# vpc-ccg/tksm

Measured on AMD Instinct MI355X. Metric: sequenced reads/s, higher is better.
Workload: dtype u8; 1 GPU; Bulk molecules, Badread error+qual model (nanopore2020, identity 84,99,5.5), 24 x 128 Mb random genome, FASTQ; kind=bulk, mean_len=1000, length_distribution=normal(1000, 200), compute_qual=True, contexts_in_flight_per_gpu=3

## Files before the change

### tksm_amd/csrc/kernels.hip

```cpp
#include "kernels.h"
#include <type_traits>

namespace tk {

#define DEV __device__ __forceinline__

constexpr int BIG = 1 << 28;
DEV bool is_inf(int v) { return v >= (1 << 27); }

struct Ph4 { uint32_t x, y, z, w; };
enum { ST_ID = 0, ST_PAD = 1, ST_IDENT = 2, ST_DRAW = 3, ST_ALNPOS = 4, ST_QUAL = 5, ST_TAIL = 6 };

DEV Ph4 philox(uint64_t seed, uint64_t read, uint32_t stream, uint32_t n) {
    uint32_t c0 = (uint32_t)read, c1 = (uint32_t)(read >> 32), c2 = stream, c3 = n;
    uint32_t k0 = (uint32_t)seed, k1 = (uint32_t)(seed >> 32);
#pragma unroll
    for (int r = 0; r < 10; r++) {
        const unsigned long long p0 = (unsigned long long)0xD2511F53u * c0, p1 = (unsigned long long)0xCD9E8D57u * c2;
        const uint32_t h0 = (uint32_t)(p0 >> 32), l0 = (uint32_t)p0, h1 = (uint32_t)(p1 >> 32), l1 = (uint32_t)p1;
        uint32_t n0 = h1 ^ c1 ^ k0, n2 = h0 ^ c3 ^ k1;
        c0 = n0; c1 = l1; c2 = n2; c3 = l0;
        k0 += 0x9E3779B9u; k1 += 0xBB67AE85u;
    }
    return Ph4{c0, c1, c2, c3};
// ... 1542 lines not shown
            }
            wave_sync();
            const int m = join_window_planar(gnb, p0, nrows, Nw, ownw, wcap, lane);
            wave_sync();
            if (m > wcap) {
                if (early_mode) { to_exact_kernel(); return; }
                break;
            }
            const AlnOut a = band_align<0, false>(Fw, nrows, Nw, ownw, m, lane, nullptr);
            st_aligns++;
            if (is_inf(a.dist)) {
                to_exact_kernel();
                return;
            }
            const int cols = (int)(a.stat & 0xffffu), mt = (int)(a.stat >> 16);
            const double ident = cols ? (double)mt / (double)cols : 0.0;
            if (L <= 1000) errors = (1.0 - ident) * frag_len;
            else {
                const double estimated = (1.0 - ident) * frag_len;
                const double weight = 1000.0 / frag_len;
                errors = estimated * weight + errors * (1.0 - weight);
            }
            aln_no++;
            st = RUN;
        }
    }
    if (lane == 0) {
        uint32_t job = 0;
        if (st == NEED_ALN) {
            job = FB.base_cur[rc] + atomicAdd(&FB.job_cnt[rc * 32u], 1u);
            st_aligns++;
            uint32_t p0 = 0, nrows = (uint32_t)L;
            if (L > 1000) {
                p0 = __umulhi(philox(P.seed, g, ST_ALNPOS, aln_no).x, (uint32_t)(L - 1000 + 1));
                nrows = 1000u;
            }
            *reinterpret_cast<uint4*>(FB.job_meta + 4ull * job) = make_uint4(r, p0, nrows, 0u);
        }
        sp->errors = errors; sp->est = est_keep; sp->change_count = change_count; sp->n_base = n; sp->aln_no = aln_no;
        sp->resume_src = -1; sp->resume_j = (int16_t)resume_j; sp->st_draws = st_draws; sp->st_aligns = st_aligns;
        sp->pending = st == NEED_ALN ? 1 : 0;
        sp->job = job;
        sp->stage = st == NEED_ALN ? 0 : 3;
        if (st == DONE) {
            atomicAdd(&FB.defer_cnt[rc * 32u], 1u);
            FB.defer_list[atomicAdd(&FB.counters[1], 1u)] = make_uint2(r, rc);
        }
    }
}

template <bool STATE_IN_HBM>
__global__ __launch_bounds__(256, 8) void k_err(BatchView B, ErrModelView EM, QsModelView QM, SimParams P, SimBuffers O,
                                              FastBuffers FB, const uint32_t* __restrict__ order, uint32_t begin, uint32_t count,
                                              int lds_lcap, int lds_ncap, int from_jobs, uint32_t c0, uint32_t c1) {
#ifndef TKSM_ABLATE
    __builtin_amdgcn_s_setprio(2);
#endif
    const int lane = threadIdx.x & 63, wave = __builtin_amdgcn_readfirstlane(threadIdx.x >> 6), wpw = blockDim.x >> 6;
    const uint32_t widx = blockIdx.x * (uint32_t)wpw + (uint32_t)wave;
    if (widx >= count) return;
    uint64_t r; uint32_t pos;
    if (!from_jobs) { pos = begin + widx; r = (uint64_t)__builtin_amdgcn_readfirstlane((int)order[pos]) & 0xffffffffull; }
    else if (from_jobs == 2) {
        const uint2 e = FB.defer_list[widx];
        r = (uint64_t)__builtin_amdgcn_readfirstlane((int)e.x) & 0xffffffffull;
        pos = (uint32_t)__builtin_amdgcn_readfirstlane((int)e.y) * FB.rs;
    } else {
        const uint32_t target = FB.prefix[c0] + widx;
        uint32_t lo2 = c0, hi2 = c1 - 1;
        while (lo2 < hi2) { const uint32_t mid = (lo2 + hi2 + 1) >> 1; if (FB.prefix[mid] <= target) lo2 = mid; else hi2 = mid - 1; }
        const uint32_t pjob = FB.base_prev[lo2] + (target - FB.prefix[lo2]);
        r = (uint64_t)__builtin_amdgcn_readfirstlane((int)FB.prev_meta[4ull * pjob]) & 0xffffffffull;
        pos = lo2 * FB.rs;
    }
    ReadState S = FB.state[r];
    if (S.stage == 2 || S.slow) return;
    if (S.stage == 0) return;
    uint16_t* gnb = nb_row(FB, r);
    const int per_wave = STATE_IN_HBM ? lds_ncap + 128 : lds_lcap * 3 + lds_ncap + 128;
    uint8_t* lds_wave = lds_raw + (size_t)wave * per_wave;
    uint8_t* frag = STATE_IN_HBM ? frag_row(FB, r) : lds_wave;
    uint16_t* nb = STATE_IN_HBM ? gnb : reinterpret_cast<uint16_t*>(lds_wave + lds_lcap);
    uint8_t* aux = STATE_IN_HBM ? lds_wave : lds_wave + 3 * (size_t)lds_lcap;
    const int k = EM.k;
    const uint64_t g = P.first_read + r * P.stride;
    const int raw_len = __builtin_amdgcn_readfirstlane(S.raw_len);
    const int L = raw_len + 2 * k;
    const uint64_t slot = O.slot_off[r];
    const int cap = __builtin_amdgcn_readfirstlane((int)((O.slot_off[r + 1] - slot) >> 1));
    uint8_t* out_seq = O.scratch + slot;
    uint8_t* out_qual = out_seq + cap;
    if (!STATE_IN_HBM) {
        const uint8_t* gfrag0 = frag_row(FB, r);
        for (int t = lane * 4; t < L; t += 256) *reinterpret_cast<uint32_t*>(frag + t) = *reinterpret_cast<const uint32_t*>(gfrag0 + t);
        for (int t = lane * 2; t < L; t += 128) *reinterpret_cast<uint32_t*>(nb + t) = *reinterpret_cast<const uint32_t*>(gnb + t);
    }
    wave_sync();
    uint32_t status = 0;
    const double frag_len = (double)L;
    const double errors = S.errors;
    const double target = S.target;
    const int change_count = __builtin_amdgcn_readfirstlane(S.change_count), st_draws = __builtin_amdgcn_readfirstlane(S.st_draws);
    int st_aligns = __builtin_amdgcn_readfirstlane(S.st_aligns);
    double identity = 1.0;

    int start_trim, end_trim;
    {
        int v1 = lane < k ? slot_len(nb[lane]) : 0, v2 = lane < k ? slot_len(nb[L - k + lane]) : 0;
        (void)prefix_small(v1, start_trim);
        (void)prefix_small(v2, end_trim);
    }
    const int jcap = min(lds_ncap, cap);
    const int m = joined_len(nb, 0, L, lane);
    int lo = start_trim, hi = end_trim == 0 ? 0 : m - end_trim;
    lo = min(lo, m); hi = max(hi, lo);
    if (m > jcap) { status |= 1; lo = hi = 0; }
    const int out_len = hi - lo;
    const bool want_q = P.compute_q && m > 0 && !(status & 1);
    if (want_q) {
        const uint32_t mt = S.res_mt, cols = S.res_cols, fail = S.res_fail;
        if (fail) { go_slow(FB, r, lane, 3); return; }
        identity = cols ? (double)mt / (double)cols : 0.0;
        const uint32_t rc1 = pos / FB.rs;
        const uint8_t* gp = FB.prev_popd + FB.geo_prev[rc1].popd_off + (size_t)(S.job - FB.base_prev[rc1]) * FB.geo_prev[rc1].ncap;
        wave_sync();
        uint8_t* popd = aux + 16;
        for (int t = lane; t < m; t += 64) popd[t] = gp[t];
        wave_sync();
        const int margins = (QM.kmer_size - 1) / 2;
        const uint32_t hmask = (uint32_t)QM.n_slots - 1u;
        for (int i2 = lo + lane; i2 < hi; i2 += 64) {
#ifdef TKSM_ABLATE
            if (P.ablate == 40) { out_qual[i2 - lo] = 40; continue; }
#endif
            const int d = max(0, max(margins - i2, i2 + margins - (m - 1)));
            int row = -1; uint32_t roff = 0, rcnt = 0;
            auto probe = [&](uint64_t key) {
                uint32_t sl = (uint32_t)qs_hash(key) & hmask;
#ifdef TKSM_ABLATE
                if (P.ablate == 41) { row = (int)(sl & 1023u); roff = 0u; rcnt = 1u; return; }
#endif
                for (;;) {
                    const uint4 e = QM.ent[sl];
                    const uint64_t kk = ((uint64_t)e.y << 32) | e.x;
                    if (kk == key) { row = (int)sl; roff = e.z; rcnt = e.w; break; }
                    if (kk == 0) break;
                    sl = (sl + 1) & hmask;
                }
            };
            if (margins <= 4) {
                const int ob = 16 + i2 - 4, sh = ob & 3;
                const uint32_t* aw = reinterpret_cast<const uint32_t*>(aux) + (ob >> 2);
                const uint32_t w0 = aw[0], w1 = aw[1], w2 = aw[2];
                const uint32_t b0 = __builtin_amdgcn_alignbyte(w1, w0, sh), b1 = __builtin_amdgcn_alignbyte(w2, w1, sh), b2 = w2 >> (8 * sh);
                auto byte_at = [&](int j) -> uint32_t { return j < 4 ? (b0 >> (8 * j)) & 255u : j < 8 ? (b1 >> (8 * (j - 4))) & 255u : b2 & 255u; };
                uint64_t K[5]; int ln[5];
                K[0] = byte_at(4) & 3u; ln[0] = 1;
#pragma unroll
                for (int h = 1; h <= 4; h++) {
                    const uint32_t bl = byte_at(4 - h);
                    const int ddl = (int)(bl >> 2), ddr = (int)(byte_at(3 + h) >> 2);
                    ln[h] = ln[h - 1] + 2 + ddl + ddr;
                    const bool fits = ln[h] <= 29;
                    const int sl_ = fits ? 2 * (1 + ddl) : 0, sr_ = fits ? 2 * (1 + ddl + ln[h - 1]) : 0, so_ = fits ? 2 * (ln[h] - 1) : 0;
                    const int dl2 = fits ? 2 * ddl : 0, dr2 = fits ? 2 * ddr : 0;
                    K[h] = (uint64_t)(bl & 3u) | (((1ull << dl2) - 1ull) << 2) | (K[h - 1] << sl_) | (((1ull << dr2) - 1ull) << sr_) |
                           ((uint64_t)(byte_at(4 + h) & 3u) << so_);
                }
                const int hmax = margins - d;
                bool pend = true;
#pragma unroll
                for (int h = 4; h >= 0; h--) {
                    const bool tryit = pend && h <= hmax;
                    if (__ballot(tryit) == 0ull) continue;
                    if (tryit && ln[h] <= 29) { probe(K[h] | ((uint64_t)ln[h] << 58)); pend = row < 0; }
#ifdef TKSM_ABLATE
                    if (P.ablate == 44) { if (row < 0) row = (int)(K[h] & 1023u); pend = false; }
                    if (P.ablate == 45 && h == 3) { if (row < 0) row = (int)(K[h] & 1023u); pend = false; }
#endif
                }
            } else {
                int s0 = i2 - margins + d, e0 = i2 + margins - d;
                for (;;) {
                    uint64_t key = 0; int len = 0; bool ok = true;
                    for (int x2 = s0; x2 <= e0; x2++) {
                        if (x2 > s0) {
                            const int dd = popd[x2 - 1] >> 2;
                            if (len + dd > 29) { ok = false; break; }
                            key |= ((1ull << (2 * dd)) - 1ull) << (2 * len); len += dd;
                        }
                        if (len >= 29) { ok = false; break; }
                        key |= (uint64_t)(popd[x2] & 3) << (2 * len); len++;
                    }
                    if (ok) probe(key | ((uint64_t)len << 58));
                    if (row >= 0 || s0 == e0) break;
                    s0++; e0--;
                }
            }
            uint8_t q = 0;
#ifdef TKSM_ABLATE
            if (P.ablate == 42) { out_qual[i2 - lo] = (uint8_t)(33 + (row & 31)); continue; }
            if (P.ablate == 43 && row >= 0) {
                const uint32_t w = (uint32_t)i2 * 2654435761u;
                const uint32_t a2 = QM.guide[(size_t)row * 64 + (w >> 26)] & 0x7fu;
                out_qual[i2 - lo] = (uint8_t)(33 + QM.pairs[roff + min(a2, rcnt - 1u)].y); continue;
            }
#endif
            if (row >= 0) {
                const uint32_t w = philox(P.seed, g, ST_QUAL, (uint32_t)i2).x;
                uint32_t a2 = QM.guide[(size_t)row * 64 + (w >> 26)];
                if (QM.guide_direct && (a2 & 0x80u)) q = (uint8_t)(a2 & 0x7fu);
                else {
                    uint2 pr = QM.pairs[roff + a2];
                    while (a2 + 1 < rcnt && !(w < pr.x)) { a2++; pr = QM.pairs[roff + a2]; }
                    q = (uint8_t)pr.y;
                }
            }
            out_qual[i2 - lo] = (uint8_t)(q + 33);
        }
    } else {
        identity = 1.0 - errors / frag_len;
    }
    join_out(frag, nb, L, out_seq, lo, hi, lane);
    if (P.quirk_perfect) identity = 1.0;
    finish_read(B, P, O, r, P.quirk_perfect ? out_len : raw_len, out_len, identity, status, st_draws, change_count, st_aligns, L, m,
                start_trim, end_trim, errors, target, lane);
    if (lane == 0) FB.state[r].stage = 2;
}

__global__ void k_collect_unfinished(FastBuffers FB, uint64_t n_reads) {
    const uint64_t r = (uint64_t)blockIdx.x * blockDim.x + threadIdx.x;
    if (r >= n_reads) return;
    ReadState S = FB.state[r];
    if (S.stage != 2 && !S.slow) {
        FB.state[r].slow = 1;
        const uint32_t idx = atomicAdd(&FB.counters[2], 1u);
        FB.slow_list[idx] = (uint32_t)r;
    }
}

DEV uint32_t range_of_job(const FastBuffers& FB, uint32_t job0) {
    uint32_t rng = 0, hi2 = FB.n_ranges - 1;
    while (rng < hi2) { const uint32_t mid = (rng + hi2 + 1) >> 1; if (FB.base_cur[mid] <= job0) rng = mid; else hi2 = mid - 1; }
    return rng;
}
__global__ __launch_bounds__(64) void k_qjobs(FastBuffers FB, int k, uint32_t count) {
    const int lane = threadIdx.x;
    const uint32_t widx = blockIdx.x * 64u + (uint32_t)lane;
    bool need = widx < count;
    uint32_t r = 0, rc = 0, job = 0;
    if (need) { const uint2 e = FB.defer_list[widx]; r = e.x; rc = e.y; }
    need = need && FB.state[r].stage == 3 && !FB.state[r].slow;
    const bool mine = need;
    unsigned long long todo = __ballot(need);
    while (todo) {
        const int leader = __builtin_ctzll(todo);
        const uint32_t lrc = (uint32_t)__shfl((int)rc, leader, 64);
        const unsigned long long grp = __ballot(need && rc == lrc);
        uint32_t base = 0;
        if (lane == leader) base = FB.base_cur[lrc] + atomicAdd(&FB.job_cnt[lrc * 32u], (uint32_t)__popcll(grp));
        base = (uint32_t)__shfl((int)base, leader, 64);
        if (need && rc == lrc) { job = base + (uint32_t)__popcll(grp & ((1ull << lane) - 1ull)); need = false; }
        todo &= ~grp;
    }
    if (mine) {
        ReadState* sp = FB.state + r;
        const uint32_t L = (uint32_t)(sp->raw_len + 2 * k);
        *reinterpret_cast<uint4*>(FB.job_meta + 4ull * job) = make_uint4(r, 0u, L | 0x80000000u, 0u);
        sp->resume_src = -1; sp->pending = 1; sp->stage = 1; sp->job = job;
    }
}

DEV int wave_max(int v) {
#pragma unroll
    for (int o = 32; o > 0; o >>= 1) v = max(v, __shfl_xor(v, o, 64));
    return v;
}
DEV void list_append(uint32_t* list, uint32_t* counter, bool want, uint32_t job, int lane) {
    const unsigned long long wm = __ballot(want);
    if (!wm) return;
    uint32_t base = 0;
    if (lane == 0) base = atomicAdd(counter, (uint32_t)__popcll(wm));
    base = __shfl(base, 0, 64);
    if (want) list[base + (uint32_t)__popcll(wm & ((1ull << lane) - 1ull))] = job;
}


constexpr uint32_t ENT_EMPTY = 0xF0000000u;
constexpr int BACKLOG_DRAIN = 20;
struct AlnJobF {
    bool act; int p0, n;
    const uint16_t* nb;
    const ulonglong2* fp; int wlast;
    unsigned long long* popd8;
};
struct AlnResF { uint32_t mt, cols; int m; bool fail, needfull, overflow; uint32_t why; };

template <int MODE, int ROWS>
DEV AlnResF aln_fused(const AlnJobF& J, uint4* trl, int tg, int cl, uint32_t ls, int mcap) {
    static_assert(ROWS == 14 || ROWS == 64, "14 stored rows, or all of them");
    constexpr int NC = ROWS == 14 ? 16 : 4;
    constexpr int ST = ROWS == 14 ? 24 : 0;
    constexpr int RAMP0 = 31 - ST;
    const bool act = J.act;
    const int n = act ? J.n : 0;
    const int base = J.p0 & ~1, skip = J.p0 - base;
    const int nmax = __builtin_amdgcn_readfirstlane(wave_max(act ? n + skip : 0));
    tg = __builtin_amdgcn_readfirstlane(tg); cl = __builtin_amdgcn_readfirstlane(cl);
    const int wb = base >> 6, bsh = base & 63;
    auto fpw = [&](int w) { return J.fp[min(max(w, 0), J.wlast)]; };
    auto aligned = [&](const ulonglong2& a, const ulonglong2& b) { ulonglong2 v; v.x = funnel128(a.x, b.x, bsh); v.y = funnel128(a.y, b.y, bsh); return v; };
    ulonglong2 Wn;
    unsigned long long A, B;
    {
        const ulonglong2 r0 = fpw(wb), r1 = fpw(wb + 1), r2 = fpw(wb + 2);
        const ulonglong2 W0 = aligned(r0, r1);
        Wn = aligned(r1, r2);
        A = ~funnel128(W0.x, Wn.x, skip); B = ~funnel128(W0.y, Wn.y, skip);
    }
    int jc = 0;
    unsigned long long EA = 0ull, EB = 0ull;
    int app = 0;
    unsigned long long Pv = ~0ull, Mv = 0ull;
    int t = 1, t32 = 1;
    uint32_t qlo = 0u, qhi = 0u;
    unsigned long long U = 0ull;
    int npend = 0, upos = 0, pcol = -1 - skip, col = 0, col32 = 0, shmax = 0;
    bool bad = false;
    struct __attribute__((packed, aligned(4))) U4b { uint32_t x, y, z, w; };
    uint32_t cw[8], cwn[8];
    auto load_codes = [&](int s, uint32_t (&d)[8]) {
        const int src = (s <= n + skip) ? base + s : base;
        const U4b* cp = reinterpret_cast<const U4b*>(J.nb + src);
        const U4b c0 = cp[0], c1 = cp[1];
        d[0] = c0.x; d[1] = c0.y; d[2] = c0.z; d[3] = c0.w; d[4] = c1.x; d[5] = c1.y; d[6] = c1.z; d[7] = c1.w;
    };
    load_codes(0, cw);
    constexpr int HS = 16;
    constexpr int LPH = HS / NC;
    uint32_t tw[16], shw[4] = {0u, 0u, 0u, 0u};
    int ql = 0;
    bool ovf = false;
    int s0 = 0;
    for (;;) {
        const bool more = s0 < nmax;
        const bool drain = __ballot(npend > (more ? BACKLOG_DRAIN : 0)) != 0ull;
        if (!more && !drain) break;
        if (ql + LPH > (ROWS == 64 ? cl : tg - 1)) { ovf = true; break; }
        if (!drain) load_codes(s0 + HS, cwn);
        const int inc = drain ? 0 : 1;
        uint4* const dl = trl + (size_t)(act ? ql : tg - 1) * ls;
        const int it0 = __builtin_amdgcn_readfirstlane(ql * NC);
        int mxn = 0, mxu = 0;
#pragma unroll
        for (int q = 0; q < HS; q++) {
            const int p = s0 + q - skip;
            const bool on = !drain && act && (uint32_t)p < (uint32_t)n;
            const uint32_t code = (cw[q >> 1] >> (16 * (q & 1))) & 0xffffu;
            const int len = on ? (int)((code >> 12) & 7u) : 0;
            const uint32_t m5 = (1u << len) - 1u;
            const uint32_t lo5 = code & m5, hi5 = (code >> 5) & m5;
            mxn = max(mxn, npend); mxu = max(mxu, upos);
            qlo |= lo5 << npend; qhi |= hi5 << npend;
            U |= (unsigned long long)(m5 << 1) << upos;
            upos += len + inc; npend += len;
            const uint32_t zz = U ? (uint32_t)__builtin_ctzll(U) : 64u;
            const int zc = (int)min(zz, (uint32_t)upos);
            pcol += zc;
            const bool have = npend > 0;
            const int used = zc + (have ? 1 : 0);
            U >>= used; upos -= used;
            uint32_t ent0 = ENT_EMPTY, ent1 = 0u, ent2 = 0u, ent3 = 0u, shb = 0xffu;
            if (have) {
                const int tn = max(1, pcol - 30);
                const uint32_t sh = (uint32_t)(tn - t);
                t = tn;
                shmax = max(shmax, (int)sh);
                const uint32_t cl = (uint32_t)__builtin_amdgcn_sbfe((int)qlo, 0u, 1u), ch = (uint32_t)__builtin_amdgcn_sbfe((int)qhi, 0u, 1u);
                qlo >>= 1; qhi >>= 1; npend--; col++;
                const bool g = t > 1;
                const uint32_t f = (sh == 0u && g) ? 1u : 0u;
                Pv = mk64(alignbit(~0u, hi32(Pv), sh), alignbit(hi32(Pv), lo32(Pv), sh) & ~f);
                Mv = mk64(hi32(Mv) >> sh, alignbit(hi32(Mv), lo32(Mv), sh) | f);
#ifdef TKSM_NO_INLINE_ASM
                {
                    const unsigned long long nA = sh >= 64u ? 0ull : (A >> sh) | (sh ? EA << (64u - sh) : 0ull), nB = sh >= 64u ? 0ull : (B >> sh) | (sh ? EB << (64u - sh) : 0ull);
                    EA = sh >= 64u ? 0ull : EA >> sh; EB = sh >= 64u ? 0ull : EB >> sh; A = nA; B = nB;
                }
#else
                {
                    uint32_t a0 = lo32(A), a1 = hi32(A), a2 = lo32(EA), a3 = hi32(EA), b0 = lo32(B), b1 = hi32(B), b2 = lo32(EB), b3 = hi32(EB);
                    asm("v_alignbit_b32 %0, %1, %0, %2" : "+v"(a0) : "v"(a1), "v"(sh));
                    asm("v_alignbit_b32 %0, %1, %0, %2" : "+v"(a1) : "v"(a2), "v"(sh));
                    asm("v_alignbit_b32 %0, %1, %0, %2" : "+v"(a2) : "v"(a3), "v"(sh));
                    asm("v_lshrrev_b32 %0, %1, %0" : "+v"(a3) : "v"(sh));
                    asm("v_alignbit_b32 %0, %1, %0, %2" : "+v"(b0) : "v"(b1), "v"(sh));
                    asm("v_alignbit_b32 %0, %1, %0, %2" : "+v"(b1) : "v"(b2), "v"(sh));
                    asm("v_alignbit_b32 %0, %1, %0, %2" : "+v"(b2) : "v"(b3), "v"(sh));
                    asm("v_lshrrev_b32 %0, %1, %0" : "+v"(b3) : "v"(sh));
                    A = mk64(a1, a0); EA = mk64(a3, a2); B = mk64(b1, b0); EB = mk64(b3, b2);
                }
#endif
                const unsigned long long clm = mk64(cl, cl), chm = mk64(ch, ch);
                const unsigned long long Eq = bool3<BOOL3(TA & (TB ^ TC))>(A ^ clm, B, chm);
                const unsigned long long Xv = Eq | Mv;
                const unsigned long long Xh = bool3<BOOL3((TA ^ TB) | TC)>((Eq & Pv) + Pv, Pv, Eq);
                const unsigned long long Ph = bool3<BOOL3(TA | ~(TB | TC))>(Mv, Xh, Pv);
                const unsigned long long Mh = Pv & Xh;
                const unsigned long long D0 = Xh | Mv;
                const unsigned long long Phs = mk64(alignbit(hi32(Ph), lo32(Ph), 31u), (lo32(Ph) << 1) | 1u);
                const unsigned long long Mhs = mk64(alignbit(hi32(Mh), lo32(Mh), 31u), lo32(Mh) << 1);
                Pv = bool3<BOOL3(TA | ~(TB | TC))>(Mhs, Xv, Phs);
                Mv = Phs & Xv;
                if constexpr (ROWS == 14) {
                    int st_s;
#ifdef TKSM_NO_INLINE_ASM
                    st_s = min(max(it0 + q, RAMP0), 31);
#else
                    asm("s_max_i32 %0, %1, %2\n\ts_min_i32 %0, %0, 31" : "=&s"(st_s) : "s"(it0 + q), "i"(RAMP0) : "scc");
#endif
                    const uint32_t st = (uint32_t)(st_s - RAMP0);
                    const uint32_t PvW = alignbit(hi32(Pv), lo32(Pv), st), PhW = alignbit(hi32(Ph), lo32(Ph), st), D0W = alignbit(hi32(D0), lo32(D0), st);
                    const uint32_t c1 = bool3<BOOL3(~(TA | TB))>(PvW, PhW, 0u);
                    const uint32_t c0 = MODE ? bool3<BOOL3(TB | (~TA & TC))>(PvW, PhW, D0W) : bool3<BOOL3(~TA & (TB | TC))>(PvW, PhW, D0W);
                    const uint32_t c1s = c1 << 14;
                    const uint32_t c01 = ((c0 & 0x3fffu) | (c1s & ~0x3fffu)) & 0x0fffffffu;
                    ent0 = c01 | (min(sh, 15u) << 28);
                } else {
                    const unsigned long long upv = Pv & ~(g ? 1ull : 0ull);
                    const unsigned long long w1 = bool3<BOOL3(~(TA | TB))>(upv, Ph, 0ull);
                    const unsigned long long w0 = MODE ? bool3<BOOL3(TB | (~TA & TC))>(upv, Ph, D0) : bool3<BOOL3(~TA & (TB | TC))>(upv, Ph, D0);
                    ent0 = lo32(w0); ent1 = hi32(w0); ent2 = lo32(w1); ent3 = hi32(w1);
                    shb = min(sh, 254u);
                }
            }
            if constexpr (ROWS == 14) {
                tw[q & 7] = ent0;
                if ((q & 7) == 7) {
                    uint4* d = dl + 128 * (q >> 3);
                    d[0] = make_uint4(tw[0], tw[1], tw[2], tw[3]); d[64] = make_uint4(tw[4], tw[5], tw[6], tw[7]);
                }
            } else {
                tw[4 * (q & 3)] = ent0; tw[4 * (q & 3) + 1] = ent1; tw[4 * (q & 3) + 2] = ent2; tw[4 * (q & 3) + 3] = ent3;
                shw[q >> 2] = (q & 3) == 0 ? shb : shw[q >> 2] | (shb << (8 * (q & 3)));
                if ((q & 3) == 3) {
                    uint4* d = dl + (act ? (size_t)(q >> 2) * ls : (size_t)0);
                    d[0] = make_uint4(tw[0], tw[1], tw[2], tw[3]); d[1] = make_uint4(tw[4], tw[5], tw[6], tw[7]);
                    d[2] = make_uint4(tw[8], tw[9], tw[10], tw[11]); d[3] = make_uint4(tw[12], tw[13], tw[14], tw[15]);
                }
            }
        }
        if constexpr (ROWS == 64) {
            const int pi = ql / LPH;
            uint4* d = act ? trl + (size_t)(cl + (pi >> 2)) * ls + (pi & 3) : trl + (size_t)(tg - 1) * ls;
            *d = make_uint4(shw[0], shw[1], shw[2], shw[3]);
        }
        bad |= mxn > 26 || mxu > 57;
        ql += LPH;
        if (ql * NC == 32) { t32 = t; col32 = col; }
        if (!drain) {
            if (s0 & 16) {
                const int ev = app - (t - 1);
                bad |= ev > 32 && s0 + HS - skip < n;
                const bool upper = ((s0 - 16) & 32) != 0;
                const bool first = s0 == 16;
                const uint32_t drop = first ? (uint32_t)skip : 0u;
                const uint32_t na = ~(upper ? hi32(Wn.x) : lo32(Wn.x)) >> drop, nb2 = ~(upper ? hi32(Wn.y) : lo32(Wn.y)) >> drop;
                EA |= (unsigned long long)na << (ev & 63); EB |= (unsigned long long)nb2 << (ev & 63);
                app += 32 - (int)drop;
                if (upper) {
                    jc++;
                    Wn = aligned(fpw(wb + jc + 1), fpw(wb + jc + 2));
                }
            }
#pragma unroll
            for (int i2 = 0; i2 < 8; i2++) cw[i2] = cwn[i2];
            s0 += HS;
        }
    }
    const int m = col;
    ovf = ovf || m > mcap;
    const uint32_t why = (bad ? 1u : 0u) | (shmax > 31 ? 8u : 0u) | (shmax > 14 ? 16u : 0u) | ((act && m > 0 && (n - t > 63 || n - t < 0)) ? 32u : 0u);
    bad = bad || (ROWS == 64 && shmax > 31);
    bool fail = act && m > 0 && (n - t > 63 || n - t < 0 || bad), needfull = ROWS == 14 && act && shmax > 14;
    bool live = act && !fail && m > 0 && !ovf && !needfull;
    uint32_t mt = 0, dg = 0;
    int bs = n - t - ST;
    int i = n, tt = t;
    int c = m - 1;
    unsigned long long acc = 0ull;
    auto walk_ent = [&](int it, auto ramp, auto lo, auto hi, uint32_t shc, bool is_col) {
        constexpr bool RAMP = decltype(ramp)::value;
        if (live && is_col) {
            if (RAMP) bs = i - tt - (min(max(it, RAMP0), 31) - RAMP0);
            uint32_t run, extra = 0u;
            if constexpr (ROWS == 64) { extra = (uint32_t)max(bs - 63, 0); bs -= (int)extra; }
            if constexpr (ROWS == 64) {
                const unsigned long long y = (lo | hi) << ((63 - bs) & 63);
                run = y ? (uint32_t)__builtin_clzll(y) : 64u;
            } else {
                const uint32_t y = (lo | hi) << ((31 - bs) & 31);
                run = y ? (uint32_t)__builtin_clz(y) : 32u;
            }
            bool ok = (uint32_t)bs < (uint32_t)ROWS;
            bool zero = false;
            if (RAMP) {
                run = min(run, (uint32_t)(bs + 1));
                if (i == 0) { run = 0u; extra = 0u; }
                zero = (uint32_t)i == run + extra || i == 0;
                ok |= i == 0;
            }
            const int bs2 = bs - (int)run;
            ok &= bs2 >= 0 || zero;
            const uint32_t lb = zero ? 1u : (uint32_t)(lo >> (bs2 & (ROWS == 64 ? 63 : 31))) & 1u;
            const uint32_t hb = zero ? 0u : (uint32_t)(hi >> (bs2 & (ROWS == 64 ? 63 : 31))) & 1u;
            needfull |= !ok;
            live = ok && !zero;
            mt += hb & lb;
            dg += hb;
            if (MODE) {
                const uint32_t op = hb ? (lb ^ 1u) : 2u;
                acc |= (unsigned long long)(op | (min(run + extra, 63u) << 2)) << (8 * (c & 7));
                if (zero) {
                    acc |= 0x0202020202020202ull & ((1ull << (8 * (c & 7))) - 1ull);
                    J.popd8[c >> 3] = acc; acc = 0ull;
                    for (int b2 = (c >> 3) - 1; b2 >= 0; b2--) J.popd8[b2] = 0x0202020202020202ull;
                } else if ((c & 7) == 0) { J.popd8[c >> 3] = acc; acc = 0ull; }
                c--;
            }
            if (RAMP) { i -= (int)(run + extra + hb); tt -= (int)shc; }
            else bs = bs2 - (int)hb + (int)shc;
        }
    };
    uint4 la0, la1, la2, la3, lb0, lb1, lb2, lb3;
    auto load_line = [&](int q, uint4& l0, uint4& l1, uint4& l2, uint4& l3) {
        const uint4* p = trl + (size_t)max(q, 0) * ls;
        if constexpr (ROWS == 14) { l0 = p[0]; l1 = p[64]; l2 = p[128]; l3 = p[192]; }
        else { l0 = p[0]; l1 = p[1]; l2 = p[2]; l3 = p[3]; }
    };
    uint4 sw = make_uint4(0u, 0u, 0u, 0u), swn = sw;
    auto load_shifts = [&](int pi) { return trl[(size_t)(cl + (max(pi, 0) >> 2)) * ls + (max(pi, 0) & 3)]; };
    auto walk_line = [&](int q, const uint4& l0, const uint4& l1, const uint4& l2, const uint4& l3) {
        const uint32_t w[16] = {l0.x, l0.y, l0.z, l0.w, l1.x, l1.y, l1.z, l1.w, l2.x, l2.y, l2.z, l2.w, l3.x, l3.y, l3.z, l3.w};
        const int cq = q * NC;
        uint32_t swq = 0u;
        if constexpr (ROWS == 64) {
            if ((q & 3) == 3) { sw = swn; swn = load_shifts((q >> 2) - 1); }
            swq = (q & 3) == 0 ? sw.x : (q & 3) == 1 ? sw.y : (q & 3) == 2 ? sw.z : sw.w;
        }
        auto ents_of_line = [&](auto ramp) {
#pragma unroll
            for (int e = NC - 1; e >= 0; e--) {
                if constexpr (ROWS == 14) {
                    const uint32_t v = w[e];
                    walk_ent(cq + e, ramp, v, v >> 14, v >> 28, v != ENT_EMPTY);
                } else {
                    const uint32_t shc = (swq >> (8 * e)) & 0xffu;
                    walk_ent(cq + e, ramp, mk64(w[4 * e + 1], w[4 * e]), mk64(w[4 * e + 3], w[4 * e + 2]), shc, shc != 0xffu);
                }
            }
        };
        if (cq >= 32) ents_of_line(std::false_type{});
        else {
            if (cq == 32 - NC && m > col32) { tt = t32; i = bs + t32 + ST; }
            ents_of_line(std::true_type{});
        }
    };
    if (ql > 0) {
        const int topq = ql - 1;
        if constexpr (ROWS == 64) swn = load_shifts(topq >> 2);
        load_line(topq, la0, la1, la2, la3);
        for (int q = topq; q >= 0; q -= 2) {
            load_line(q - 1, lb0, lb1, lb2, lb3);
            walk_line(q, la0, la1, la2, la3);
            if (q > 0) {
                load_line(q - 2, la0, la1, la2, la3);
                walk_line(q - 1, lb0, lb1, lb2, lb3);
            }
        }
    }
    AlnResF R;
    R.mt = mt; R.cols = (uint32_t)(n + m) - dg; R.m = m;
    R.fail = fail || (ROWS == 64 && needfull); R.needfull = ROWS != 64 && needfull; R.overflow = act && ovf;
    R.why = why | (needfull ? 64u : 0u) | ((uint32_t)min(max(bs + 8, 0), 255) << 8);
    return R;
}

DEV void load_job_f(const FastBuffers& FB, uint32_t job, uint32_t rng, bool act, AlnJobF& J, uint32_t& r, int& mcap) {
    J.act = act;
    r = 0;
    J.p0 = 0; J.n = 0;
    if (act) {
        const uint4 meta = *reinterpret_cast<const uint4*>(FB.job_meta + 4ull * job);
        r = meta.x; J.p0 = (int)meta.y; J.n = (int)(meta.z & 0x7fffffffu);
    }
    const RangeGeo G = FB.geo_cur[rng];
    const uint32_t rel = job - FB.base_cur[rng];
    J.nb = nb_row(FB, r);
    J.fp = reinterpret_cast<const ulonglong2*>(planes_row(FB, r));
    J.wlast = planes_words(FB, r) - 1;
    J.popd8 = reinterpret_cast<unsigned long long*>(FB.job_popd + G.popd_off + (size_t)rel * G.ncap);
    mcap = (int)G.ncap;
}
DEV void job_overflow(const FastBuffers& FB, const SimBuffers& O, uint32_t r) {
    O.status[r] |= 1u; O.out_len[r] = 0; O.rec_len[r] = 0; O.identity[r] = 0.0;
    FB.state[r].stage = 2;
}
DEV void store_result_f(const FastBuffers& FB, uint32_t r, const AlnResF& R) {
    ReadState* st = FB.state + r;
    st->res_mt = R.mt; st->res_cols = R.cols; st->res_fail = (R.fail || R.needfull) ? 1u : 0u;
}

constexpr int ALNF_WAVES = 4;
constexpr int LONG_QJOB = 3000;
#ifdef TKSM_ALNF_NUM_VGPR
#define ALNF_VGPR_CAP __attribute__((amdgpu_num_vgpr(TKSM_ALNF_NUM_VGPR)))
#else
#define ALNF_VGPR_CAP
#endif
template <int MODE, int ROWS, bool LIST>
__global__ __launch_bounds__(64, ROWS == 64 ? 3 : ALNF_WAVES) ALNF_VGPR_CAP void k_alnf(SimParams P, FastBuffers FB, SimBuffers O, uint32_t n_jobs) {
#ifndef TKSM_ABLATE
    if (ROWS == 64) __builtin_amdgcn_s_setprio(2);
#endif
    const int lane = threadIdx.x;
    if (!LIST) {
        const uint32_t job0 = blockIdx.x * 64u, job = job0 + (uint32_t)lane;
        const uint32_t rng = range_of_job(FB, job0);
        const uint32_t rbase = FB.base_cur[rng];
        const uint32_t in_rng = FB.job_cnt[rng * 32u];
        if (in_rng <= job0 - rbase) return;
        AlnJobF J;
        uint32_t r;
        bool act = job < n_jobs && job - rbase < in_rng;
        uint4* trl;
        int tg, mcap;
        bool norow = false;
        uint32_t ls = 256u;
        if (ROWS == 64) {
            const unsigned long long wm = __ballot(act);
            const uint32_t na = (uint32_t)__popcll(wm);
            uint32_t base = 0;
            if (lane == 0) base = atomicAdd(&FB.counters[3], na);
            base = (uint32_t)__builtin_amdgcn_readfirstlane((int)base);
            if (base + na > FB.full_rows) { norow = act; act = false; base = 0; }
            tg = (int)FB.full_tg;
            ls = 4u * max(na, 1u);
            trl = reinterpret_cast<uint4*>(FB.trace_full) + ((size_t)base * FB.full_tg + (uint32_t)__popcll(wm & ((1ull << lane) - 1ull)) % max(na, 1u)) * 4;
        } else {
            const RangeGeo G = FB.geo_cur[rng];
            const uint32_t rel = job - rbase;
            tg = (int)G.tstride;
            trl = reinterpret_cast<uint4*>(FB.trace) + (G.trace_off + (size_t)(rel >> 6) * G.tstride * 64) * 4 + (rel & 63u);
        }
        load_job_f(FB, job, rng, act || norow, J, r, mcap);
        const bool straight_to_list = MODE == 1 && ROWS == 14 && act && J.n > LONG_QJOB;
        J.act = act && !straight_to_list;
        AlnResF R = aln_fused<MODE, ROWS>(J, trl, tg, (int)FB.full_cl, ls, mcap);
        if (straight_to_list) { R.fail = false; R.needfull = true; R.overflow = false; }
        if (norow) { R.fail = true; R.needfull = false; R.overflow = false; }
        if (act && R.overflow) { job_overflow(FB, O, r); return; }
        if (ROWS != 64) list_append(FB.redo_list, FB.counters + 10, act && R.needfull, job, lane);
        if ((act || norow) && !R.needfull) store_result_f(FB, r, R);
        if (act && R.fail) { atomicAdd(&FB.counters[12], 1u); atomicOr(&FB.counters[13], R.why & 255u); FB.counters[14] = R.why; FB.counters[15] = (uint32_t)J.n | ((uint32_t)R.m << 16);
              for (int b = 0; b < 8; b++) if ((R.why >> b) & 1u) atomicAdd(&FB.counters[16 + b], 1u); if (MODE) atomicAdd(&FB.counters[24], 1u); if (LIST) atomicAdd(&FB.counters[25], 1u); }
    } else {
        static_assert(!LIST || ROWS == 64, "the list holds the jobs of the full-width pass");
        const uint32_t n_list = FB.counters[10];
        if (lane == 0 && blockIdx.x == 0 && n_list) { atomicAdd(&FB.counters[8], n_list); atomicAdd(&FB.counters[9], (n_list + 63u) / 64u); }
        const uint32_t* list = FB.redo_list;
        const int tg = (int)FB.full_tg;
        uint4* trl = reinterpret_cast<uint4*>(FB.trace_full) + ((size_t)blockIdx.x * tg * 64 + (uint32_t)lane) * 4;
        for (uint32_t base = blockIdx.x * 64u; base < n_list; base += gridDim.x * 64u) {
            const uint32_t idx = base + (uint32_t)lane;
            const bool act = idx < n_list;
            const uint32_t job = list[min(idx, n_list - 1u)];
            const uint32_t rng = range_of_job(FB, job);
            AlnJobF J;
            uint32_t r;
            int mcap;
            load_job_f(FB, job, rng, act, J, r, mcap);
            const AlnResF R = aln_fused<MODE, ROWS>(J, trl, tg, (int)FB.full_cl, 256u, mcap);
            if (act && R.overflow) job_overflow(FB, O, r);
            else if (act) store_result_f(FB, r, R);
            if (act && R.fail) { atomicAdd(&FB.counters[12], 1u); atomicOr(&FB.counters[13], R.why & 255u); FB.counters[14] = R.why; FB.counters[15] = (uint32_t)J.n | ((uint32_t)R.m << 16);
              for (int b = 0; b < 8; b++) if ((R.why >> b) & 1u) atomicAdd(&FB.counters[16 + b], 1u); if (MODE) atomicAdd(&FB.counters[24], 1u); if (LIST) atomicAdd(&FB.counters[25], 1u); }
        }
    }
}

DEV int put_str(uint8_t* o, const char* s) { int n = 0; while (s[n]) { o[n] = (uint8_t)s[n]; n++; } return n; }
DEV int put_u(uint8_t* o, unsigned long long v) {
    int d = ndigits(v);
    for (int i = d - 1; i >= 0; i--) { o[i] = (uint8_t)('0' + v % 10); v /= 10; }
    return d;
}

DEV int format_header(uint8_t* hdr, const SimParams& P, uint64_t g, uint32_t out_len, uint32_t raw_len, double identity) {
    int kx = 0;
    hdr[kx++] = P.fastq ? '@' : '>';
    const Ph4 id = philox(P.seed, g, ST_ID, 0);
    const uint32_t w[4] = {id.x, id.y, id.z, id.w};
    int nib = 0;
    for (int a = 0; a < 4; a++)
        for (int b = 7; b >= 0; b--) {
            if (nib == 8 || nib == 12 || nib == 16 || nib == 20) hdr[kx++] = '-';
            const uint32_t v = (w[a] >> (4 * b)) & 15u;
            hdr[kx++] = (uint8_t)(v < 10 ? '0' + v : 'a' + v - 10); nib++;
        }
    kx += put_str(hdr + kx, " length="); kx += put_u(hdr + kx, out_len);
    kx += put_str(hdr + kx, " error_free_length="); kx += put_u(hdr + kx, raw_len);
    kx += put_str(hdr + kx, " read_identity=");
    const long long h = pct_hundredths(identity);
    kx += put_u(hdr + kx, (unsigned long long)(h / 100));
    hdr[kx++] = '.'; hdr[kx++] = (uint8_t)('0' + (h % 100) / 10); hdr[kx++] = (uint8_t)('0' + h % 10);
    kx += put_str(hdr + kx, "% molecule_id=");
    return kx;
}

DEV void flush_image(const uint8_t* img, int a, uint32_t rec_len, uint8_t* gout , int lane) {
    const uint32_t end = (uint32_t)a + rec_len;
    const uint32_t c0 = a ? 1u : 0u, c1 = end >> 4;
    for (uint32_t c = c0 + lane; c < c1; c += 64) *reinterpret_cast<uint4*>(gout + 16u * c) = *reinterpret_cast<const uint4*>(img + 16u * c);
    if (lane < 2) {
        const uint32_t lo = lane == 0 ? (uint32_t)a : max(16u * c1, (uint32_t)a), hi = lane == 0 ? (a ? min(16u, end) : 0u) : end;
        for (uint32_t t = lo; t < hi; t++) gout[t] = img[t];
    }
}

constexpr int EMIT_IMG = 6144;

__global__ __launch_bounds__(256, 6) void k_emit(BatchView B, SimParams P, SimBuffers O, const uint64_t* __restrict__ rec_off,
                                               uint8_t* __restrict__ records) {
    __shared__ __attribute__((aligned(16))) uint8_t img_all[WAVES_PER_WG][EMIT_IMG + 32];
    __shared__ uint8_t hdr_all[WAVES_PER_WG][160];
#ifndef TKSM_ABLATE
    __builtin_amdgcn_s_setprio(2);
#endif
    const int lane = threadIdx.x & 63, wave = threadIdx.x >> 6;
    const uint64_t r = (uint64_t)blockIdx.x * WAVES_PER_WG + wave;
    if (r >= B.n_reads) return;
    uint8_t* hdr = hdr_all[wave];
    const uint64_t g = P.first_read + r * P.stride;
    const uint32_t out_len = O.out_len[r], raw_len = P.quirk_perfect ? O.out_len[r] : O.raw_len[r] - (O.tail_len ? O.tail_len[r] : 0u);
    int hl = 0;
    if (lane == 0) hl = format_header(hdr, P, g, out_len, raw_len, O.identity[r]);
    hl = __shfl(hl, 0, 64);
    wave_sync();
    const uint64_t off = rec_off[r], rec_len = rec_off[r + 1] - off;
    const uint32_t ido = B.ids[2 * r], idl = B.ids[2 * r + 1];
    const uint8_t* seq = O.scratch + O.slot_off[r];
    const uint64_t cap = (O.slot_off[r + 1] - O.slot_off[r]) >> 1;
    const bool real_q = P.mode == 1 && P.compute_q && !P.quirk_perfect;
    const uint8_t* qual = seq + cap;
    const int a = (int)(reinterpret_cast<uintptr_t>(records + off) & 15);
    if (rec_len + (uint64_t)a > (uint64_t)EMIT_IMG) {
        uint8_t* dst = records + off;
        for (int t = lane; t < hl; t += 64) dst[t] = hdr[t];
        dst += hl;
        for (uint32_t t = lane; t < idl; t += 64) dst[t] = B.idpool[ido + t];
        dst += idl;
        if (lane == 0) dst[0] = '\n';
        dst += 1;
        for (uint32_t t = lane; t < out_len; t += 64) dst[t] = seq[t];
        dst += out_len;
        if (lane == 0) dst[0] = '\n';
        dst += 1;
        if (P.fastq) {
            if (lane == 0) { dst[0] = '+'; dst[1] = '\n'; }
            dst += 2;
            for (uint32_t t = lane; t < out_len; t += 64) dst[t] = real_q ? qual[t] : (uint8_t)'K';
            dst += out_len;
            if (lane == 0) dst[0] = '\n';
        }
        return;
    }
    uint8_t* img = img_all[wave];
    for (int t = lane; t < hl; t += 64) img[a + t] = hdr[t];
    for (uint32_t t = lane; t < idl; t += 64) img[a + hl + t] = B.idpool[ido + t];
    if (lane == 0) img[a + hl + idl] = '\n';
    uint8_t* simg = img + a + hl + idl + 1;
    for (uint32_t t0 = 16u * lane; t0 < out_len; t0 += 1024u) {
        const uint4 v = *reinterpret_cast<const uint4*>(seq + t0);
        __builtin_memcpy(simg + t0, &v, 16);
    }
    wave_sync();
    if (lane == 0) { simg[out_len] = '\n'; if (P.fastq) { simg[out_len + 1] = '+'; simg[out_len + 2] = '\n'; } }
    if (P.fastq) {
        uint8_t* qimg = simg + out_len + 3;
        for (uint32_t t0 = 16u * lane; t0 < out_len; t0 += 1024u) {
            uint4 v = make_uint4(0x4b4b4b4bu, 0x4b4b4b4bu, 0x4b4b4b4bu, 0x4b4b4b4bu);
            if (real_q) v = *reinterpret_cast<const uint4*>(qual + t0);
            __builtin_memcpy(qimg + t0, &v, 16);
        }
        wave_sync();
        if (lane == 0) qimg[out_len] = '\n';
    }
    wave_sync();
    flush_image(img, a, (uint32_t)rec_len, records + off - a, lane);
}

__global__ void k_perfect_lengths(BatchView B, RefView R, SimParams P, SimBuffers O) {
    const uint64_t r = (uint64_t)blockIdx.x * blockDim.x + threadIdx.x;
    if (r >= B.n_reads) return;
    const uint32_t L = O.raw_len[r], idl = B.ids[2 * r + 1];
    uint32_t status = 0;
    const uint32_t ib = B.reads[2 * r], ic = B.reads[2 * r + 1];
    for (uint32_t ii = 0; ii < ic; ii++) {
        const Ivl iv = load_interval(B, R, ib + ii);
        for (uint32_t mi = iv.mod_begin; mi < iv.mod_end; mi++)
            if (B.mods[2ull * mi] >= iv.len) status |= 2;
    }
    if (status) O.status[r] |= status;
    uint64_t rec = 1 + 36 + 8 + ndigits(L) + 19 + ndigits(L) + 15 + 3 + 3 + 14 + idl + 1;
    rec += (uint64_t)L + 1;
    if (P.fastq) rec += 2 + (uint64_t)L + 1;
    O.out_len[r] = L; O.identity[r] = 1.0; O.rec_len[r] = rec;
}

DEV void perfect_record_bytewise(const BatchView& B, const RefView& R, const SimParams& P, uint64_t r, uint32_t L, uint8_t* hdr,
                                 uint8_t* dst, int lane) {
    int hl = 0;
    wave_sync();
    if (lane == 0) hl = format_header(hdr, P, P.first_read + r * P.stride, L, L, 1.0);
    hl = __shfl(hl, 0, 64);
    wave_sync();
    for (int t = lane; t < hl; t += 64) dst[t] = hdr[t];
    dst += hl;
    const uint32_t ido = B.ids[2 * r], idl = B.ids[2 * r + 1];
    for (uint32_t t = lane; t < idl; t += 64) dst[t] = B.idpool[ido + t];
    dst += idl;
    if (lane == 0) dst[0] = '\n';
    dst += 1;
    const uint32_t ib = B.reads[2 * r], ic = B.reads[2 * r + 1];
    for (uint32_t ii = 0; ii < ic; ii++) {
        const Ivl iv = load_interval(B, R, ib + ii);
        const uint32_t len = iv.len;
        for (uint32_t t = lane; t < len; t += 64) {
            const uint32_t src = iv.minus ? len - 1 - t : t;
            uint8_t b = iv.literal ? upper(B.litpool[iv.gbase + iv.s + src]) : ref_base(R, iv.gbase + iv.s + src);
            for (uint32_t mi = iv.mod_begin; mi < iv.mod_end; mi++)
                if (B.mods[2ull * mi] == src) b = (uint8_t)B.mods[2ull * mi + 1];
            dst[t] = iv.minus ? comp(b) : b;
        }
        dst += len;
    }
    if (lane == 0) dst[0] = '\n';
    dst += 1;
    if (P.fastq) {
        if (lane == 0) { dst[0] = '+'; dst[1] = '\n'; }
        dst += 2;
        for (uint32_t t = lane; t < L; t += 64) dst[t] = (uint8_t)'K';
        dst += L;
        if (lane == 0) dst[0] = '\n';
    }
}

__constant__ char PERFECT_TEXT[] = " length= error_free_length= read_identity=100.00% molecule_id=";
constexpr int PT_LEN = 8, PT_EFL = 19, PT_REST = 35;
constexpr int PERFECT_IMG_MAX = 8192;
constexpr int PERFECT_IMG_LONG = 36864;
constexpr int PERFECT_IVLS = 32;
struct PIvl { unsigned long long g; uint32_t len, o, pc, flags, mod_begin, mod_end; };
int perfect_lds_bytes(int img_bytes) { return WAVES_PER_WG * (img_bytes + 32 + PERFECT_IVLS * (int)sizeof(PIvl) + 160); }

#ifndef PERFECT_WAVES
#define PERFECT_WAVES 5
// ... 418 lines not shown
```

Baseline: 15.17 million reads/s.

## Align code loads to 64-byte boundaries and load two half-steps per fetch

Aligns the read base position to a multiple of 32 codes instead of 2, so each code fetch is a 64-byte-aligned uint4 load. Codes are now loaded once every other 16-step block into a 16-word buffer, which cuts the number of global loads. Because skip can now be as large as 31, the ramp region of the banded alignment is shifted by skip and extended from 32 to 64 columns in both the forward pass and the traceback. It also simplifies the entry packing, dropping the clamp of the shift to 15 and using a plain min/max in place of scalar inline asm. The larger skip lengthens the ramp and the padding work, and removing the shift clamp could corrupt entries if sh ever exceeds 15.

After: 15.13 million reads/s. About the same (-0.3%).

```diff
diff --git a/tksm_amd/csrc/kernels.hip b/tksm_amd/csrc/kernels.hip
--- a/tksm_amd/csrc/kernels.hip
+++ b/tksm_amd/csrc/kernels.hip
@@ -1868,9 +1868,11 @@
     constexpr int NC = ROWS == 14 ? 16 : 4;
     constexpr int ST = ROWS == 14 ? 24 : 0;
     constexpr int RAMP0 = 31 - ST;
+    constexpr int RAMPN = 64;
     const bool act = J.act;
     const int n = act ? J.n : 0;
-    const int base = J.p0 & ~1, skip = J.p0 - base;
+    const int base = J.p0 & ~31, skip = J.p0 - base;
+    const int ramp_off = skip + RAMP0;
     const int nmax = __builtin_amdgcn_readfirstlane(wave_max(act ? n + skip : 0));
     tg = __builtin_amdgcn_readfirstlane(tg); cl = __builtin_amdgcn_readfirstlane(cl);
     const int wb = base >> 6, bsh = base & 63;
@@ -1891,17 +1893,19 @@
     int t = 1, t32 = 1;
     uint32_t qlo = 0u, qhi = 0u;
     unsigned long long U = 0ull;
-    int npend = 0, upos = 0, pcol = -1 - skip, col = 0, col32 = 0, shmax = 0;
+    int npend = 0, upos = 0, pcol = -1 - skip, col = 0, col32 = 0x7fffffff, shmax = 0;
     bool bad = false;
-    struct __attribute__((packed, aligned(4))) U4b { uint32_t x, y, z, w; };
-    uint32_t cw[8], cwn[8];
-    auto load_codes = [&](int s, uint32_t (&d)[8]) {
-        const int src = (s <= n + skip) ? base + s : base;
-        const U4b* cp = reinterpret_cast<const U4b*>(J.nb + src);
-        const U4b c0 = cp[0], c1 = cp[1];
-        d[0] = c0.x; d[1] = c0.y; d[2] = c0.z; d[3] = c0.w; d[4] = c1.x; d[5] = c1.y; d[6] = c1.z; d[7] = c1.w;
+    uint32_t cw[8], cln[16];
+    auto load_codes = [&](int s) {
+        const int src = (s < n + skip) ? base + s : base;
+        const uint4* cp = reinterpret_cast<const uint4*>(J.nb + src);
+        const uint4 c0 = cp[0], c1 = cp[1], c2 = cp[2], c3 = cp[3];
+        cln[0] = c0.x; cln[1] = c0.y; cln[2] = c0.z; cln[3] = c0.w; cln[4] = c1.x; cln[5] = c1.y; cln[6] = c1.z; cln[7] = c1.w;
+        cln[8] = c2.x; cln[9] = c2.y; cln[10] = c2.z; cln[11] = c2.w; cln[12] = c3.x; cln[13] = c3.y; cln[14] = c3.z; cln[15] = c3.w;
     };
-    load_codes(0, cw);
+    load_codes(0);
+#pragma unroll
+    for (int i2 = 0; i2 < 8; i2++) cw[i2] = cln[i2];
     constexpr int HS = 16;
     constexpr int LPH = HS / NC;
     uint32_t tw[16], shw[4] = {0u, 0u, 0u, 0u};
@@ -1913,7 +1917,7 @@
         const bool drain = __ballot(npend > (more ? BACKLOG_DRAIN : 0)) != 0ull;
         if (!more && !drain) break;
         if (ql + LPH > (ROWS == 64 ? cl : tg - 1)) { ovf = true; break; }
-        if (!drain) load_codes(s0 + HS, cwn);
+        if (!drain && (s0 & 16)) load_codes(s0 + HS);
         const int inc = drain ? 0 : 1;
         uint4* const dl = trl + (size_t)(act ? ql : tg - 1) * ls;
         const int it0 = __builtin_amdgcn_readfirstlane(ql * NC);
@@ -1979,19 +1983,11 @@
                 Pv = bool3<BOOL3(TA | ~(TB | TC))>(Mhs, Xv, Phs);
                 Mv = Phs & Xv;
                 if constexpr (ROWS == 14) {
-                    int st_s;
-#ifdef TKSM_NO_INLINE_ASM
-                    st_s = min(max(it0 + q, RAMP0), 31);
-#else
-                    asm("s_max_i32 %0, %1, %2\n\ts_min_i32 %0, %0, 31" : "=&s"(st_s) : "s"(it0 + q), "i"(RAMP0) : "scc");
-#endif
-                    const uint32_t st = (uint32_t)(st_s - RAMP0);
+                    const uint32_t st = (uint32_t)min(max(it0 + q - ramp_off, 0), ST);
                     const uint32_t PvW = alignbit(hi32(Pv), lo32(Pv), st), PhW = alignbit(hi32(Ph), lo32(Ph), st), D0W = alignbit(hi32(D0), lo32(D0), st);
                     const uint32_t c1 = bool3<BOOL3(~(TA | TB))>(PvW, PhW, 0u);
                     const uint32_t c0 = MODE ? bool3<BOOL3(TB | (~TA & TC))>(PvW, PhW, D0W) : bool3<BOOL3(~TA & (TB | TC))>(PvW, PhW, D0W);
-                    const uint32_t c1s = c1 << 14;
-                    const uint32_t c01 = ((c0 & 0x3fffu) | (c1s & ~0x3fffu)) & 0x0fffffffu;
-                    ent0 = c01 | (min(sh, 15u) << 28);
+                    ent0 = (c0 & 0x3fffu) | ((c1 & 0x3fffu) << 14) | (sh << 28);
                 } else {
                     const unsigned long long upv = Pv & ~(g ? 1ull : 0ull);
                     const unsigned long long w1 = bool3<BOOL3(~(TA | TB))>(upv, Ph, 0ull);
@@ -2023,7 +2019,7 @@
         }
         bad |= mxn > 26 || mxu > 57;
         ql += LPH;
-        if (ql * NC == 32) { t32 = t; col32 = col; }
+        if (ql * NC == RAMPN) { t32 = t; col32 = col; }
         if (!drain) {
             if (s0 & 16) {
                 const int ev = app - (t - 1);
@@ -2038,9 +2034,12 @@
                     jc++;
                     Wn = aligned(fpw(wb + jc + 1), fpw(wb + jc + 2));
                 }
-            }
-#pragma unroll
-            for (int i2 = 0; i2 < 8; i2++) cw[i2] = cwn[i2];
+#pragma unroll
+                for (int i2 = 0; i2 < 8; i2++) cw[i2] = cln[i2];
+            } else {
+#pragma unroll
+                for (int i2 = 0; i2 < 8; i2++) cw[i2] = cln[8 + i2];
+            }
             s0 += HS;
         }
     }
@@ -2058,7 +2057,7 @@
     auto walk_ent = [&](int it, auto ramp, auto lo, auto hi, uint32_t shc, bool is_col) {
         constexpr bool RAMP = decltype(ramp)::value;
         if (live && is_col) {
-            if (RAMP) bs = i - tt - (min(max(it, RAMP0), 31) - RAMP0);
+            if (RAMP) bs = i - tt - min(max(it - ramp_off, 0), ST);
             uint32_t run, extra = 0u;
             if constexpr (ROWS == 64) { extra = (uint32_t)max(bs - 63, 0); bs -= (int)extra; }
             if constexpr (ROWS == 64) {
@@ -2126,9 +2125,9 @@
                 }
             }
         };
-        if (cq >= 32) ents_of_line(std::false_type{});
+        if (cq >= RAMPN) ents_of_line(std::false_type{});
         else {
-            if (cq == 32 - NC && m > col32) { tt = t32; i = bs + t32 + ST; }
+            if (cq == RAMPN - NC && m > col32) { tt = t32; i = bs + t32 + ST; }
             ents_of_line(std::true_type{});
         }
     };
```
